# fixie-ai/ultravox

Measured on NVIDIA H100. Metric: audio-sec/s prefill (Llama-3.1-8B, 30s clip) at 1/2/4/8 H100; TTFT p50, higher is better.
Workload: dtype bf16

## Files before the change

### include/uvx.h

```cpp
#ifndef UVX_H_
#define UVX_H_

#include <stddef.h>
#include <stdint.h>

#ifdef __cplusplus
extern "C" {
#endif

#define UVX_ABI_VERSION 1

#define UVX_OK 0
#define UVX_ERR_ARG (-1)
#define UVX_ERR_CUDA (-2)
#define UVX_ERR_WS (-3)

typedef void* uvx_stream_t;

int uvx_abi_version(void);
const char* uvx_last_error(void);
int64_t uvx_launch_count(void);

size_t uvx_logmel_workspace(int64_t B, int64_t L, int n_mels);
int uvx_logmel(const float* wave, int64_t B, int64_t L, int n_mels, float* out_f32, void* out_tm,
               void* workspace, size_t workspace_bytes, uvx_stream_t stream);

int uvx_debug_mel_filters(int n_mels, float* host_dense);

int uvx_mel_to_timemajor(const float* mel, int64_t N, int n_mels, int64_t T, void* out_tm, uvx_stream_t stream);

enum { UVX_ACT_NONE = 0, UVX_ACT_GELU = 1, UVX_ACT_SWIGLU = 2 };
enum { UVX_DT_BF16 = 0, UVX_DT_F32 = 1 };
enum { UVX_TILE_PLAIN = 0, UVX_TILE_ROPE_PAIRS = 1, UVX_TILE_GATE_UP_8 = 8, UVX_TILE_GATE_UP_16 = 16 };

typedef struct uvx_gemm_args {
  const void* A;
  int64_t a_batch, a_rows, K;
  int64_t a_row_stride, a_batch_stride;
  const void* W;
  int64_t N, w_row_stride;
  void* C;
  int64_t c_row_stride, c_batch_rows, c_row_offset;
  const int32_t* c_row_map;
  const void* bias;
  const void* R;
  int64_t r_row_stride, r_batch_stride;
  float alpha;
  int32_t act;
  int32_t out_dtype;
  void* workspace;
  int64_t workspace_bytes;
  const void* norm_w;
  void* norm_out;
  float norm_eps;
  int32_t w_tiled;
  int32_t rope_cols;
  const float* rope_cos;
  const float* rope_sin;
  const int32_t* rope_positions;
  int64_t rope_rows_per_seq, rope_pos_offset;
  int32_t flags;
  int32_t w_perm;
} uvx_gemm_args;

int uvx_gemm_bf16(const uvx_gemm_args* args, uvx_stream_t stream);
int uvx_debug_gemm_override(int cfg, int splits);
int uvx_debug_gemm_stages(int n);
int uvx_debug_gemm_ws(int enable, int mode, int grid);
int uvx_debug_gemm_tma_store(int on);
int uvx_debug_gemm_times(void* dev_buf);
int uvx_debug_gemm_pf(int pf);
int uvx_debug_gemm_ws_times(void* dev_buf);
int uvx_tile_weight(const void* W, int64_t N, int64_t K, int64_t w_row_stride, int32_t R, int32_t interleave, void* out,
                    uvx_stream_t stream);
int uvx_debug_gemm_cluster(int cm, int cn);
int uvx_debug_gemm_mode(int mode);

int uvx_layernorm(const void* x, const void* w, const void* b, void* y, int64_t rows, int64_t cols,
                  int64_t x_row_stride, float eps, uvx_stream_t stream);
int uvx_rmsnorm(const void* x, const void* w, void* y, int64_t rows, int64_t cols, int64_t x_row_stride,
                int64_t group_rows, int64_t group_stride, int64_t valid_elems, float eps, uvx_stream_t stream);

typedef struct uvx_attn_args {
  const void *q, *k, *v;
  void* o;
  int64_t B, Hq, Hkv, Sq, Skv, D;
  int64_t q_rs, q_bs, k_rs, k_bs, v_rs, v_bs, o_rs, o_bs;
  const int32_t* kv_len;
  int32_t causal;
  int32_t block;
  float scale;
  float* lse;
// ... 144 lines not shown
```

### ultravox_b200/_lib.py

```python
from __future__ import annotations

import ctypes as C
import os
import pathlib

_HERE = pathlib.Path(__file__).resolve().parent
LIB_PATH = _HERE / "libuvx.so"

c_i64, c_i32, c_f32, c_vp, c_sz = C.c_int64, C.c_int32, C.c_float, C.c_void_p, C.c_size_t


class GemmArgs(C.Structure):
    _fields_ = [("A", c_vp), ("a_batch", c_i64), ("a_rows", c_i64), ("K", c_i64), ("a_row_stride", c_i64),
                ("a_batch_stride", c_i64), ("W", c_vp), ("N", c_i64), ("w_row_stride", c_i64), ("C", c_vp),
                ("c_row_stride", c_i64), ("c_batch_rows", c_i64), ("c_row_offset", c_i64), ("c_row_map", c_vp),
                ("bias", c_vp), ("R", c_vp), ("r_row_stride", c_i64), ("r_batch_stride", c_i64), ("alpha", c_f32),
                ("act", c_i32), ("out_dtype", c_i32), ("workspace", c_vp), ("workspace_bytes", c_i64),
                ("norm_w", c_vp), ("norm_out", c_vp), ("norm_eps", c_f32), ("w_tiled", c_i32), ("rope_cols", c_i32),
                ("rope_cos", c_vp), ("rope_sin", c_vp), ("rope_positions", c_vp), ("rope_rows_per_seq", c_i64),
                ("rope_pos_offset", c_i64), ("flags", c_i32), ("w_perm", c_i32)]


class AttnArgs(C.Structure):
    _fields_ = [("q", c_vp), ("k", c_vp), ("v", c_vp), ("o", c_vp), ("B", c_i64), ("Hq", c_i64), ("Hkv", c_i64),
# ... 7 lines not shown


class TensorList(C.Structure):
    _fields_ = [("count", c_i64), ("numel", c_i64 * TL_MAX), ("g", c_vp * TL_MAX), ("acc", c_vp * TL_MAX), ("p", c_vp * TL_MAX),
                ("m", c_vp * TL_MAX), ("v", c_vp * TL_MAX)]


SIGNATURES = {
    "uvx_abi_version": (C.c_int, []),
    "uvx_last_error": (C.c_char_p, []),
    "uvx_launch_count": (c_i64, []),
    "uvx_logmel_workspace": (c_sz, [c_i64, c_i64, C.c_int]),
    "uvx_logmel": (C.c_int, [c_vp, c_i64, c_i64, C.c_int, c_vp, c_vp, c_vp, c_sz, c_vp]),
    "uvx_debug_mel_filters": (C.c_int, [C.c_int, c_vp]),
    "uvx_mel_to_timemajor": (C.c_int, [c_vp, c_i64, C.c_int, c_i64, c_vp, c_vp]),
    "uvx_gemm_bf16": (C.c_int, [C.POINTER(GemmArgs), c_vp]),
    "uvx_debug_gemm_override": (C.c_int, [C.c_int, C.c_int]),
    "uvx_debug_gemm_cluster": (C.c_int, [C.c_int, C.c_int]),
    "uvx_debug_gemm_mode": (C.c_int, [C.c_int]),
    "uvx_debug_gemm_pf": (C.c_int, [C.c_int]),
    "uvx_debug_gemm_stages": (C.c_int, [C.c_int]),
    "uvx_debug_gemm_times": (C.c_int, [c_vp]),
    "uvx_debug_gemm_tma_store": (C.c_int, [C.c_int]),
    "uvx_debug_gemm_ws": (C.c_int, [C.c_int, C.c_int, C.c_int]),
    "uvx_debug_gemm_ws_times": (C.c_int, [C.c_void_p]),
    "uvx_tile_weight": (C.c_int, [c_vp, c_i64, c_i64, c_i64, c_i32, c_i32, c_vp, c_vp]),
    "uvx_layernorm": (C.c_int, [c_vp, c_vp, c_vp, c_vp, c_i64, c_i64, c_i64, c_f32, c_vp]),
    "uvx_rmsnorm": (C.c_int, [c_vp, c_vp, c_vp, c_i64, c_i64, c_i64, c_i64, c_i64, c_i64, c_f32, c_vp]),
    "uvx_attention": (C.c_int, [C.POINTER(AttnArgs), c_vp]),
    "uvx_debug_attn_tc": (C.c_int, [C.c_int]),
    "uvx_attention_enc_tc": (C.c_int, [c_vp, c_i64, c_i64, c_i64, c_i64, c_i64, c_i64, c_i64, c_vp, c_i64, c_vp, c_i32, c_f32, c_vp]),
    "uvx_attention_indexed": (C.c_int, [C.POINTER(AttnArgs), c_i64, c_vp, c_vp, c_vp]),
    "uvx_attention_paged": (C.c_int, [C.POINTER(AttnArgs), c_vp, c_i64, c_vp]),
    "uvx_attention_indexed_paged": (C.c_int, [C.POINTER(AttnArgs), c_i64, c_vp, c_i64, c_vp, c_vp, c_vp]),
    "uvx_kv_page_map": (C.c_int, [c_vp, c_i64, c_vp, c_vp, c_vp, c_i64, c_i64, c_vp, c_vp, c_vp]),
    "uvx_kv_pages_copy": (C.c_int, [c_vp, c_vp, c_i64, c_vp, c_vp, c_i64, c_i64, c_i64, c_vp, c_i64, c_i64, c_i32, c_vp]),
    "uvx_rope": (C.c_int, [c_vp, c_i64, c_i64, C.c_int, C.c_int, C.c_int, c_vp, c_vp, c_vp, c_i64, c_i64, c_vp]),
    "uvx_swiglu": (C.c_int, [c_vp, c_vp, c_i64, c_i64, c_i64, C.c_int, c_vp]),
    "uvx_splice_plan": (C.c_int, [c_vp, c_vp, c_vp, c_i64, c_i64, c_i64, c_i64, c_vp, c_vp]),
    "uvx_embed_splice": (C.c_int, [c_vp, c_vp, c_i64, c_vp, c_vp, c_i64, c_i64, c_vp, c_vp]),
    "uvx_lm_head": (C.c_int, [c_vp, c_i64, c_i64, c_vp, c_i64, c_i64, c_vp, c_vp]),
    "uvx_gemv_bf16": (C.c_int, [c_vp, c_i64, c_i64, c_vp, c_i64, c_i64, c_i64, c_vp, c_i64, c_vp, c_i64, C.c_int, c_vp]),
    "uvx_kv_append": (C.c_int, [c_vp, c_i64, c_i64, c_i64, c_i64, c_vp, c_vp, c_i64, c_vp, c_i64, c_vp]),
    "uvx_gemv_fused_bf16": (C.c_int, [c_vp, c_i64, c_i64, c_vp, c_i64, c_i64, c_i64, c_vp, c_i64, c_vp, c_i64, C.c_int, c_vp, C.c_float,
                                      C.c_int, c_vp]),
    "uvx_rope_kv_append": (C.c_int, [c_vp, c_i64, c_i64, C.c_int, C.c_int, C.c_int, c_vp, c_vp, c_vp, c_vp, c_vp, c_i64, c_vp, c_vp]),
# ... 74 lines not shown
```

### ultravox_b200/csrc/gemm_tc.cu

```cuda
#include <stdlib.h>

#include "uvx_common.cuh"
#include "tc_ptx.cuh"

namespace uvx {

struct GemmParams {
  int64_t a_rows, a_batch, K, N;
  void* C;
  int64_t c_row_stride, c_batch_rows, c_row_offset;
  const int32_t* c_row_map;
  const bf16* bias;
  const bf16* R;
  int64_t r_row_stride, r_batch_stride;
  float alpha;
  int act, out_f32;
  int m_tiles;
  int n_tiles, num_tiles;
  int splits, kb_per_split;
  float* ws_partial;
  const bf16* norm_w;
  bf16* norm_out;
  float norm_eps;
  int w_tiled;
  int w_perm;
  int swiglu;
  const float* rope_cos;
  const float* rope_sin;
  const int32_t* rope_pos;
  int64_t rope_rows_per_seq, rope_pos_offset;
  int rope_cols;
  int stages;
  int cm, cn;
  int staged_bytes;
  int r_bcast;
};

static constexpr int kSmemTotal = 227 * 1024;
static constexpr int kMaxStages = 8;
static constexpr int kGemmThreads = 384;
static constexpr int kPanelBytes = 128 * 128;

template <int MT, int BN>
struct WgLayout {
  static constexpr int kABytes = MT * 128 * kBK * 2;
  static constexpr int kWBytes = BN * kBK * 2;
  static constexpr int kStageBytes = kABytes + kWBytes;
  static constexpr int kRingMax = kSmemTotal - 1024 - 256;
  static constexpr int kStages = kRingMax / kStageBytes > kMaxStages ? kMaxStages : kRingMax / kStageBytes;
  static constexpr int kAcc = BN / 2;
  static_assert(kStages >= 2, "ring too shallow");
  static_assert(MT * kAcc <= 128, "accumulators must fit the register file");
};

__device__ __forceinline__ int tile_col(int tc, int perm) {
  if (!perm) return tc;
  const int q = tc >> 5, j = tc & 31;
  return j < 16 ? 16 * q + j : 64 + 16 * q + (j - 16);
}

__device__ __forceinline__ int64_t out_row(const GemmParams& p, int b, int64_t m) {
  return p.c_row_map ? (int64_t)p.c_row_map[(int64_t)b * p.a_rows + m] : (int64_t)b * p.c_batch_rows + m + p.c_row_offset;
}

template <int BN, int I>
__device__ __forceinline__ void swiglu_row(const GemmParams& p, const float* a, int h, int cq, bf16* crow, int64_t n_out0) {
#pragma unroll
  for (int j = 0; j < BN / 8; ++j) {
    if ((8 * j) % (2 * I) >= I) continue;
    const int64_t f = n_out0 + (8 * j / (2 * I)) * I + (8 * j) % (2 * I) + cq;
    if (f >= p.N / 2) continue;
// ... 8 lines not shown
    *reinterpret_cast<__nv_bfloat162*>(crow + f) = __floats2bfloat162_rn(o[0], o[1]);
  }
}

__device__ __forceinline__ void rope_store(const GemmParams& p, float x1a, float x1b, float x2a, float x2b, int64_t pos, int d, bf16* crow) {
  const float2 cs = *reinterpret_cast<const float2*>(p.rope_cos + pos * 64 + d);
  const float2 sn = *reinterpret_cast<const float2*>(p.rope_sin + pos * 64 + d);
  float o1a, o2a, o1b, o2b;
  rope_pair(__bfloat162float(__float2bfloat16_rn(x1a * p.alpha)), __bfloat162float(__float2bfloat16_rn(x2a * p.alpha)), cs.x, sn.x, o1a, o2a);
  rope_pair(__bfloat162float(__float2bfloat16_rn(x1b * p.alpha)), __bfloat162float(__float2bfloat16_rn(x2b * p.alpha)), cs.y, sn.y, o1b, o2b);
  *reinterpret_cast<__nv_bfloat162*>(crow + d) = __floats2bfloat162_rn(o1a, o1b);
  *reinterpret_cast<__nv_bfloat162*>(crow + d + 64) = __floats2bfloat162_rn(o2a, o2b);
}

template <int MT, int BN, bool STAGED>
__global__ void __launch_bounds__(kGemmThreads, 1)
gemm_wg_kernel(const __grid_constant__ CUtensorMap tmA, const __grid_constant__ CUtensorMap tmW, const __grid_constant__ CUtensorMap tmC,
               const __grid_constant__ CUtensorMap tmR, const GemmParams p) {
  using L = WgLayout<MT, BN>;
  static_assert(!STAGED || (MT == 1 && BN <= 128), "the staged epilogue is built for 128 x 64 and 128 x 128 tiles");
  pdl_trigger();
  extern __shared__ uint8_t smem_raw[];
  uint8_t* smem = (uint8_t*)(((uintptr_t)smem_raw + 1023) & ~(uintptr_t)1023);
  uint8_t* stage_c = smem + p.stages * L::kStageBytes;
  uint64_t* full_bar = (uint64_t*)(stage_c + p.staged_bytes);
  uint64_t* empty_bar = full_bar + kMaxStages;
  uint64_t* res_full = empty_bar + kMaxStages;
  uint64_t* stage_free = res_full + 1;

  const int wg = threadIdx.x >> 7, tid = threadIdx.x & 127;
  const int tiles_m_total = p.m_tiles * (int)p.a_batch;
  const int num_kb = (int)((p.K + kBK - 1) / kBK);
  const int stages = p.stages;
  const int cm = STAGED ? 1 : p.cm, cn = STAGED ? 1 : p.cn;
  const int csize = cm * cn;
  const int rank = csize > 1 ? (int)cluster_ctarank() : 0;
  const int rm = rank / cn, rn = rank % cn;
  const int cluster_tiles_m = tiles_m_total / cm;
  const int num_units = p.num_tiles / csize * p.splits;
  const int first_unit = blockIdx.x / csize, unit_step = gridDim.x / csize;

  if (threadIdx.x == 0) {
    for (int s = 0; s < stages; ++s) {
      mbar_init(&full_bar[s], 1);
      mbar_init(&empty_bar[s], 8 * csize);
    }
    if (STAGED) {
      mbar_init(res_full, 1);
      mbar_init(stage_free, 1);
    }
    asm volatile("fence.mbarrier_init.release.cluster;" ::: "memory");
    asm volatile("fence.proxy.async.shared::cta;" ::: "memory");
  }
  if (csize > 1) cluster_sync();
  else __syncthreads();
  pdl_wait();

  if (wg == 0) {
    asm volatile("setmaxnreg.dec.sync.aligned.u32 40;");
    if (tid == 0) {
      asm volatile("prefetch.tensormap [%0];" ::"l"(&tmA) : "memory");
      asm volatile("prefetch.tensormap [%0];" ::"l"(&tmW) : "memory");
      const int a_slice = MT * 128 / cn, w_slice = BN / cm;
      const uint16_t row_mask = (uint16_t)(((1u << cn) - 1u) << (rm * cn));
      uint16_t col_mask = 0;
      for (int j = 0; j < cm; ++j) col_mask |= (uint16_t)(1u << (j * cn + rn));
      int s = 0;
      uint32_t ph = 0;
      for (int unit = first_unit, tile_i = 0; unit < num_units; unit += unit_step, ++tile_i) {
        const int ctile = unit / p.splits, split = unit % p.splits;
        const int tm_idx = (ctile % cluster_tiles_m) * cm + rm;
        const int tn_idx = (ctile / cluster_tiles_m) * cn + rn;
        const int b = tm_idx / p.m_tiles;
        const int m0 = (tm_idx % p.m_tiles) * (MT * 128);
        const int kb_begin = split * p.kb_per_split;
        const int kb_end = min(num_kb, kb_begin + p.kb_per_split);
        const int wt_base = tn_idx * num_kb * BN;
        const int r_kb = max(kb_begin, kb_end - stages);
        for (int kb = kb_begin; kb < kb_end; ++kb) {
          mbar_wait(&empty_bar[s], ph ^ 1u);
          uint8_t* sa = smem + s * L::kStageBytes;
          mbar_expect_tx(&full_bar[s], (uint32_t)L::kStageBytes);
          uint8_t* da = sa + rn * a_slice * (kBK * 2);
          if (cn > 1) tma_load_3d_mc(da, &tmA, kb * kBK, m0 + rn * a_slice, b, &full_bar[s], row_mask);
          else tma_load_3d(da, &tmA, kb * kBK, m0, b, &full_bar[s]);
          uint8_t* dw = sa + L::kABytes + rm * w_slice * (kBK * 2);
          const int w0 = p.w_tiled ? 0 : kb * kBK;
          const int w1 = (p.w_tiled ? wt_base + kb * BN : tn_idx * BN) + rm * w_slice;
          if (cm > 1) tma_load_2d_mc(dw, &tmW, w0, w1, &full_bar[s], col_mask);
          else tma_load_2d(dw, &tmW, w0, w1, &full_bar[s]);
          if (++s == stages) { s = 0; ph ^= 1u; }
          if (STAGED && p.R && kb == r_kb) {
            mbar_wait(stage_free, (uint32_t)(tile_i & 1) ^ 1u);
            const int n0 = tn_idx * BN, panels = (int)min((int64_t)BN, p.N - n0) / 64;
            mbar_expect_tx(res_full, (uint32_t)(panels * kPanelBytes));
            for (int q = 0; q < panels; ++q) tma_load_3d(stage_c + q * kPanelBytes, &tmR, n0 + 64 * q, m0, p.r_bcast ? 0 : b, res_full);
          }
        }
      }
    }
    if (csize > 1) cluster_sync();
    return;
  }

  asm volatile("setmaxnreg.inc.sync.aligned.u32 232;");
  const int c = wg - 1;
  const int warp = tid >> 5, lane = tid & 31;
  auto release = [&](int slot) {
    __syncwarp();
    if (csize == 1) {
      if (lane == 0) mbar_arrive(&empty_bar[slot]);
    } else if (lane < csize) {
      mbar_arrive_cluster(&empty_bar[slot], (uint32_t)lane);
    }
  };
  auto store_thread = [&]() { return STAGED && threadIdx.x == 128; };
  int s = 0;
  uint32_t ph = 0;
  for (int unit = first_unit; unit < num_units; unit += unit_step) {
    const int ctile = unit / p.splits, split = unit % p.splits;
    const int tm_idx = (ctile % cluster_tiles_m) * cm + rm;
    const int tn_idx = (ctile / cluster_tiles_m) * cn + rn;
    const int b = tm_idx / p.m_tiles;
    const int m0 = (tm_idx % p.m_tiles) * (MT * 128);
    const int n0 = tn_idx * BN;
    const int kb_begin = split * p.kb_per_split;
    const int kb_end = min(num_kb, kb_begin + p.kb_per_split);

    float acc[MT][L::kAcc];
    int prev = -1;
    for (int kb = kb_begin; kb < kb_end; ++kb) {
      mbar_wait(&full_bar[s], ph);
      const uint32_t sa = smem_u32(smem + s * L::kStageBytes);
      const uint64_t dw = make_wgmma_desc(sa + L::kABytes);
      wgmma_fence();
#pragma unroll
      for (int mt = 0; mt < MT; ++mt) {
        const uint64_t da = make_wgmma_desc(sa + (mt * 128 + c * 64) * (kBK * 2));
#pragma unroll
        for (int k = 0; k < kBK / 16; ++k)
          Wgmma<BN>::mma(acc[mt], da + (uint64_t)(2 * k), dw + (uint64_t)(2 * k), (kb > kb_begin || k > 0) ? 1u : 0u);
      }
      wgmma_commit();
      if (store_thread() && kb == kb_begin && unit != first_unit) {
        bulk_wait_read0();
        mbar_arrive(stage_free);
      }
      wgmma_wait<1>();
      if (prev >= 0) release(prev);
      prev = s;
      if (++s == stages) { s = 0; ph ^= 1u; }
    }
    wgmma_wait<0>();
    release(prev);

    const int rq = warp * 16 + (lane >> 2);
    const int cq = 2 * (lane & 3);
    if constexpr (STAGED) {
      {
        const uint32_t tile_par = (uint32_t)((unit - first_unit) / unit_step) & 1u;
        if (p.R) mbar_wait(res_full, tile_par);
        else mbar_wait(stage_free, tile_par ^ 1u);
        __nv_bfloat162 bias_v[BN / 8];
#pragma unroll
        for (int j = 0; j < BN / 8; ++j) {
          const int64_t n = n0 + 8 * j + cq;
          if (p.bias && n < p.N) bias_v[j] = *reinterpret_cast<const __nv_bfloat162*>(p.bias + n);
        }
        const uint32_t st0 = smem_u32(stage_c);
#pragma unroll
        for (int h = 0; h < 2; ++h) {
          const int r = c * 64 + rq + 8 * h;
          const uint32_t row = st0 + (uint32_t)r * 128u, sw = (uint32_t)(r & 7);
#pragma unroll
          for (int j = 0; j < BN / 8; ++j) {
            float v0 = acc[0][4 * j + 2 * h] * p.alpha, v1 = acc[0][4 * j + 2 * h + 1] * p.alpha;
            if (p.bias) {
// ... 455 lines not shown
                   CU_TENSOR_MAP_INTERLEAVE_NONE, CU_TENSOR_MAP_SWIZZLE_128B, promo, CU_TENSOR_MAP_FLOAT_OOB_FILL_NONE);
  if (r != CUDA_SUCCESS) {
    set_error("cuTensorMapEncodeTiled failed with CUresult %d (rank %d dims %llu %llu stride %llu)", (int)r, rank,
              (unsigned long long)dims[0], (unsigned long long)dims[1], (unsigned long long)strides_bytes[0]);
    return UVX_ERR_CUDA;
  }
  return UVX_OK;
}

static int num_sms() {
  static int n = 0;
  if (!n) {
    int dev = 0;
    cudaGetDevice(&dev);
    cudaDeviceGetAttribute(&n, cudaDevAttrMultiProcessorCount, dev);
    if (n <= 0) n = 132;
  }
  return n;
}

static int g_gemm_stage_cap = 0;
static int g_grid_cap = 0;
static int g_tma_store = -1;

static int finish_gemm(const uvx_gemm_args* a, const GemmParams& p, cudaStream_t stream) {
  const bool want_norm = a->norm_w && a->norm_out;
  if (p.splits == 1) {
    if (!want_norm) return UVX_OK;
    return uvx_rmsnorm(a->C, a->norm_w, a->norm_out, a->a_batch * a->a_rows, a->N, a->c_row_stride, 0, 0, 0, a->norm_eps, stream);
  }
  if (want_norm && !p.out_f32 && a->N <= 8192 && !a->c_row_map && a->act == UVX_ACT_NONE) {
    launch_k(splitk_reduce_rmsnorm_kernel, dim3((unsigned)(a->a_batch * a->a_rows)), dim3(256), 0, stream, p);
    return check_launch("splitk_reduce_rmsnorm_kernel");
  }
  const int64_t total = a->a_batch * a->a_rows * (a->N / 8);
  int64_t blocks = (total + 255) / 256;
  if (blocks > (int64_t)num_sms() * 8) blocks = (int64_t)num_sms() * 8;
  launch_k(splitk_reduce_kernel, dim3((unsigned)blocks), dim3(256), 0, stream, p);
  int rc = check_launch("splitk_reduce_kernel");
  if (rc || !want_norm) return rc;
  return uvx_rmsnorm(a->C, a->norm_w, a->norm_out, a->a_batch * a->a_rows, a->N, a->c_row_stride, 0, 0, 0, a->norm_eps, stream);
}

static void legal_cluster(int mt, int bn, int tiles_m_total, int n_tiles, int* cm, int* cn) {
  if (*cm < 1 || *cm > 4 || tiles_m_total % *cm != 0 || bn % (8 * *cm) != 0) *cm = 1;
  if (*cn < 1 || *cn > 4 || n_tiles % *cn != 0 || (mt * 128) % (8 * *cn) != 0) *cn = 1;
  if (*cm * *cn > 8) *cm = *cn = 1;
}

template <int MT, int BN, bool STAGED>
static cudaError_t set_smem_attr() {
  if constexpr (STAGED && !(MT == 1 && BN <= 128)) return cudaErrorInvalidValue;
  else return cudaFuncSetAttribute(gemm_wg_kernel<MT, BN, STAGED>, cudaFuncAttributeMaxDynamicSharedMemorySize, kSmemTotal);
}

template <int MT, int BN>
static int launch_gemm(const uvx_gemm_args* a, int splits, int cm, int cn, cudaStream_t stream) {
  using L = WgLayout<MT, BN>;
  const int m_tiles = (int)((a->a_rows + MT * 128 - 1) / (MT * 128));
  const int n_tiles = (int)((a->N + BN - 1) / BN);
  legal_cluster(MT, BN, m_tiles * (int)a->a_batch, n_tiles, &cm, &cn);
  CUtensorMap tmA, tmW;
  {
    uint64_t dims[3] = {(uint64_t)a->K, (uint64_t)a->a_rows, (uint64_t)a->a_batch};
    uint64_t st[2] = {(uint64_t)a->a_row_stride * 2, (uint64_t)(a->a_batch > 1 ? a->a_batch_stride : a->a_row_stride) * 2};
    uint32_t box[3] = {kBK, (uint32_t)(MT * 128 / cn), 1};
    int rc = encode_map(&tmA, a->A, 3, dims, st, box, CU_TENSOR_MAP_L2_PROMOTION_L2_128B);
    if (rc) return rc;
  }
  const bool tiled = a->w_tiled != 0;
  if (tiled) {
    UVX_REQUIRE(a->w_tiled == BN && a->K % kBK == 0, "uvx_gemm_bf16: tiled weights need BN == tile rows and K %% 64 == 0");
    const uint64_t n_tiles_w = (uint64_t)((a->N + BN - 1) / BN);
    uint64_t dims[2] = {(uint64_t)kBK, n_tiles_w * (uint64_t)(a->K / kBK) * (uint64_t)BN};
    uint64_t st[1] = {(uint64_t)kBK * 2};
    uint32_t box[2] = {kBK, (uint32_t)(BN / cm)};
    int rc = encode_map(&tmW, a->W, 2, dims, st, box, CU_TENSOR_MAP_L2_PROMOTION_L2_256B);
    if (rc) return rc;
  } else {
    uint64_t dims[2] = {(uint64_t)a->K, (uint64_t)a->N};
    uint64_t st[1] = {(uint64_t)a->w_row_stride * 2};
    uint32_t box[2] = {kBK, (uint32_t)(BN / cm)};
    int rc = encode_map(&tmW, a->W, 2, dims, st, box, CU_TENSOR_MAP_L2_PROMOTION_L2_256B);
    if (rc) return rc;
  }
  GemmParams p;
  memset(&p, 0, sizeof(p));
  p.w_tiled = tiled ? 1 : 0;
  p.w_perm = a->w_perm == 1 ? 1 : 0;
// ... 9 lines not shown
  p.a_batch = a->a_batch;
  p.K = a->K;
  p.N = a->N;
  p.C = a->C;
  p.c_row_stride = a->c_row_stride;
  p.c_batch_rows = a->c_batch_rows;
  p.c_row_offset = a->c_row_offset;
  p.c_row_map = a->c_row_map;
  p.bias = (const bf16*)a->bias;
  p.R = (const bf16*)a->R;
  p.r_row_stride = a->r_row_stride;
  p.r_batch_stride = a->r_batch_stride;
  p.alpha = a->alpha;
  p.act = a->act;
  p.out_f32 = a->out_dtype == UVX_DT_F32;
  p.norm_w = (const bf16*)a->norm_w;
  p.norm_out = (bf16*)a->norm_out;
  p.norm_eps = a->norm_eps;
  p.m_tiles = m_tiles;
  p.n_tiles = n_tiles;
  p.num_tiles = p.m_tiles * (int)a->a_batch * p.n_tiles;
  p.cm = cm;
  p.cn = cn;
  const int num_kb = (int)((a->K + kBK - 1) / kBK);
  if (a->N % BN != 0) splits = 1;
  const size_t per_split = (size_t)a->a_batch * (size_t)a->a_rows * (size_t)a->N * 4;
  while (splits > 1 && (!a->workspace || per_split * (size_t)splits > (size_t)a->workspace_bytes)) --splits;
  if (splits > num_kb) splits = num_kb;
  if (splits < 1) splits = 1;
  p.kb_per_split = (num_kb + splits - 1) / splits;
  p.splits = (num_kb + p.kb_per_split - 1) / p.kb_per_split;
  p.ws_partial = (float*)a->workspace;
  CUtensorMap tmC, tmR;
  memset(&tmC, 0, sizeof(tmC));
  memset(&tmR, 0, sizeof(tmR));
  const bool staged = MT == 1 && BN <= 128 && g_tma_store != 0 && (a->a_rows > 256 || a->a_batch > 1) && p.splits == 1 &&
                      cm * cn == 1 && !a->c_row_map && !p.swiglu && !p.rope_cos && !p.w_perm && !(a->norm_w && a->norm_out) &&
                      (!a->R || (!p.out_f32 && a->r_row_stride > 0 && (uintptr_t)a->R % 16 == 0));
  if (staged) {
    const uint64_t es = p.out_f32 ? 4 : 2;
    const uint64_t row_bytes = (uint64_t)a->c_row_stride * es;
    uint64_t dims[3] = {(uint64_t)a->N, (uint64_t)a->a_rows, (uint64_t)a->a_batch};
    uint64_t st[2] = {row_bytes, a->a_batch > 1 ? (uint64_t)a->c_batch_rows * row_bytes : row_bytes};
    uint32_t box[3] = {(uint32_t)(128 / es), 128, 1};
    int rc = encode_map(&tmC, (const char*)a->C + a->c_row_offset * (int64_t)row_bytes, 3, dims, st, box,
                        CU_TENSOR_MAP_L2_PROMOTION_NONE, p.out_f32 ? CU_TENSOR_MAP_DATA_TYPE_FLOAT32 : CU_TENSOR_MAP_DATA_TYPE_BFLOAT16);
    if (rc) return rc;
    if (a->R) {
      p.r_bcast = a->a_batch == 1 || a->r_batch_stride == 0;
      uint64_t rdims[3] = {(uint64_t)a->N, (uint64_t)a->a_rows, p.r_bcast ? 1 : (uint64_t)a->a_batch};
      uint64_t rst[2] = {(uint64_t)a->r_row_stride * 2, (uint64_t)(p.r_bcast ? a->r_row_stride : a->r_batch_stride) * 2};
      uint32_t rbox[3] = {64, 128, 1};
      rc = encode_map(&tmR, a->R, 3, rdims, rst, rbox, CU_TENSOR_MAP_L2_PROMOTION_L2_128B);
      if (rc) return rc;
    }
    p.staged_bytes = BN / 64 * (p.out_f32 ? 2 : 1) * kPanelBytes;
  }
  p.stages = (L::kRingMax - p.staged_bytes) / L::kStageBytes;
  if (p.stages > L::kStages) p.stages = L::kStages;
  if (g_gemm_stage_cap >= 2 && p.stages > g_gemm_stage_cap) p.stages = g_gemm_stage_cap;
  const int smem = p.stages * L::kStageBytes + p.staged_bytes + 1024 + 2 * kMaxStages * 8 + 16;
  static bool attr_set[2] = {false, false};
  if (!attr_set[staged]) {
    cudaError_t e = staged ? set_smem_attr<MT, BN, true>() : set_smem_attr<MT, BN, false>();
    if (e != cudaSuccess) {
      set_error("cudaFuncSetAttribute(gemm_wg_kernel<%d,%d,%d>, smem %d): %s", MT, BN, (int)staged, kSmemTotal, cudaGetErrorString(e));
      return UVX_ERR_CUDA;
    }
    attr_set[staged] = true;
  }
  const int csize = cm * cn;
  const int units = p.num_tiles / csize * p.splits;
  int max_units = num_sms();
  if (csize > 1) {
    static int max_clusters[9] = {0};
    if (!max_clusters[csize]) {
      cudaLaunchConfig_t cfg = {};
      cfg.gridDim = dim3((unsigned)csize);
      cfg.blockDim = dim3(kGemmThreads);
      cfg.dynamicSmemBytes = (size_t)smem;
      cudaLaunchAttribute attr;
      attr.id = cudaLaunchAttributeClusterDimension;
      attr.val.clusterDim.x = (unsigned)csize;
      attr.val.clusterDim.y = 1;
// ... 159 lines not shown
extern "C" int uvx_debug_gemm_stages(int n) {
  uvx::g_gemm_stage_cap = n;
  return UVX_OK;
}

extern "C" int uvx_debug_gemm_ws(int enable, int mode, int grid) {
  (void)mode;
  uvx::g_ws_enable = enable;
  uvx::g_grid_cap = grid > 0 ? grid : 0;
  return UVX_OK;
}

static int forced_cm = 0, forced_cn = 0;
static int g_cluster_enable = -1;

extern "C" int uvx_debug_gemm_cluster(int cm, int cn) {
  forced_cm = cm;
  forced_cn = cn;
  return UVX_OK;
}

extern "C" int uvx_debug_gemm_tma_store(int on) {
  uvx::g_tma_store = on;
  return UVX_OK;
}

extern "C" int uvx_debug_gemm_mode(int mode) { (void)mode; return UVX_OK; }
extern "C" int uvx_debug_gemm_times(void* dev_buf) { (void)dev_buf; return UVX_OK; }
extern "C" int uvx_debug_gemm_pf(int pf) { (void)pf; return UVX_OK; }
extern "C" int uvx_debug_gemm_ws_times(void* dev_buf) { (void)dev_buf; return UVX_OK; }

static void read_forced() {
  if (forced < 0) {
    const char* e = getenv("UVX_GEMM_CFG");
    forced = e ? atoi(e) : 0;
    const char* s = getenv("UVX_GEMM_SPLITS");
    forced_splits = s ? atoi(s) : 0;
  }
}

static void pick_cfg(int64_t rows, int64_t batch, int64_t N, int64_t K, int sms, int* mt_out, int* bn_out, int* splits) {
  const int num_kb = (int)((K + 63) / 64);
  int mt, bn;
  if (rows <= 256 && batch == 1) {
    mt = rows > 128 ? 2 : 1;
    bn = N % 128 == 0 ? 128 : 64;
// ... 107 lines not shown
```

### ultravox_b200/model.py

```python
from __future__ import annotations

import dataclasses
import os
from typing import Optional

import torch
import torch.nn as nn
from transformers.modeling_outputs import CausalLMOutputWithPast

from . import ops
from .config import LossConfig, LossFunction, UltravoxConfig

FUSE_NORM = os.environ.get("UVX_FUSE_NORM", "1") != "0"
USE_TILED = os.environ.get("UVX_TILED", "1") != "0"
FUSE_ROPE = os.environ.get("UVX_FUSE_ROPE", "1") != "0"
QKV_MODE = os.environ.get("UVX_QKV_MODE", "fused")
TILED_SET = os.environ.get("UVX_TILED_SET", "gate_up")
USE_WS = os.environ.get("UVX_GEMM_WS", "0") == "1"
FUSE_SWIGLU = os.environ.get("UVX_FUSE_SWIGLU", "1") != "0"
BF16 = torch.bfloat16


class _P(nn.Module):

# ... 378 lines not shown
    @torch.no_grad()
    def _tiled_weights(self):
        if getattr(self, "_tiled", None) is None:
            self._tiled = False
            layers = self.language_model.model.layers
            if USE_TILED and len(layers) > 0 and layers[0].self_attn.qkv_w.is_cuda:
                tc = self.config.text_config
                hs, ffn = tc.hidden_size, tc.intermediate_size
                per_layer = 2 * (layers[0].self_attn.qkv_w.numel() + hs * layers[0].self_attn.o_proj.weight.shape[1] + 3 * hs * ffn)
                free, _ = torch.cuda.mem_get_info(self.device)
                if hs % 64 == 0 and ffn % 64 == 0 and ffn % 8 == 0 and free > 1.15 * per_layer * len(layers) + (8 << 30):
                    out = []
                    for layer in layers:
                        sa, mlp = layer.self_attn, layer.mlp
                        attn_t = USE_WS or TILED_SET == "all"
                        down_t = USE_WS or TILED_SET in ("all", "mlp")
                        gu_rows = 128
                        lm_hd = self.language_model.head_dim
                        out.append(dict(qkv=ops.TiledWeight(sa.qkv_w, 128, rope_pairs=USE_WS and lm_hd == 128) if attn_t else None,
                                        o=ops.TiledWeight(sa.o_proj.weight, 128) if attn_t else None,
                                        gate_up=ops.TiledWeight(mlp.gate_up_w, gu_rows, swiglu=True) if FUSE_SWIGLU
                                        else ops.TiledWeight(mlp.gate_up_w, gu_rows),
                                        down=ops.TiledWeight(mlp.down_proj.weight, 128) if down_t else None))
                    self._tiled = out
        return self._tiled or None

    def _rope_tables(self, need: int):
        have = 0 if self._rope is None else self._rope[0].shape[0]
        if have < need:
            cap = int(getattr(self.config.text_config, "max_position_embeddings", 0) or 0)
            n = max(need, 4096, 2 * have)
            if cap >= need:
                n = min(n, cap)
            self._rope = ops.rope_tables(self._inv_freq, n, self.device)
        return self._rope

    def encode_audio(self, x_tm: torch.Tensor, audio_lens: Optional[torch.Tensor],
                     kv_len: Optional[torch.Tensor] = None) -> torch.Tensor:
        at = self.audio_tower
        N, Tp, _ = x_tm.shape
        T = Tp - 2
        if T > at.max_context_length:
            raise ValueError(f"Whisper expects the mel input features to be of length {at.max_context_length} or less, "
                             f"but found {T}. Make sure to pad the input mel features to {at.max_context_length}.")
        d, H = at.d, at.heads
        T2 = (T + 1) // 2
# ... 91 lines not shown
        dev = inputs_embeds.device
        past = cache.length if cache is not None else 0
        cos, sin = self._rope_tables(past + S)
        h = inputs_embeds.view(B * S, Dm)
        x = torch.empty_like(h)
        qkv = torch.empty(B * S, (nq + 2 * nkv) * hd, dtype=BF16, device=dev)
        att = torch.empty(B * S, nq * hd, dtype=BF16, device=dev)
        ffn = tc.intermediate_size
        tiled = self._tiled_weights()
        if USE_WS and B * S > 256:
            tiled = None
        fuse_act = tiled is not None and tiled[0]["gate_up"].swiglu
        gu = None if fuse_act else torch.empty(B * S, 2 * ffn, dtype=BF16, device=dev)
        act = torch.empty(B * S, ffn, dtype=BF16, device=dev)
        rs = qkv.stride(0)
        layers = lm.model.layers
        rope = (cos, sin, positions, S, past, (nq + nkv) * hd) if (FUSE_ROPE and QKV_MODE == "fused" and hd == 128) else None
        qkv_flags = 1 if QKV_MODE == "r1" else 0
        ops.rmsnorm(h, layers[0].input_layernorm.weight, eps, out=x)
        for li, layer in enumerate(layers):
            sa, mlp = layer.self_attn, layer.mlp
            tw = tiled[li] if tiled is not None else None
            if tw is not None and tw["qkv"] is not None:
                ops.linear_tiled(x, tw["qkv"], out=qkv, rope=rope)
            else:
                ops.linear(x, sa.qkv_w, out=qkv, rope=rope, flags=qkv_flags)
            if rope is None:
                ops.rope_(qkv, nq, nkv, hd, cos, sin, rows_per_seq=S, pos_offset=past, positions=positions)
            if cache is None:
                ops.attention_fused_qkv(qkv, B, S, nq, nkv, hd, hd ** -0.5, True, kv_len, 0, out=att, kv_start=kv_start)
            else:
                kc, vc = cache.k[li], cache.v[li]
                ops.kv_write(qkv, kc, vc, B, S, past, nq, nkv, hd)
                smax = kc.shape[1]
                ops.attention(qkv.data_ptr(), kc.data_ptr(), vc.data_ptr(), att, B, nq, nkv, S, past + S, hd,
                              (rs, S * rs, nkv * hd, smax * nkv * hd, nkv * hd, smax * nkv * hd, nq * hd, S * nq * hd),
                              hd ** -0.5, True, kv_len, 0, kv_start)
            n1 = (layer.post_attention_layernorm.weight, eps, x) if FUSE_NORM else None
            if tw is not None and tw["o"] is not None:
                ops.linear_tiled(att, tw["o"], residual=h, out=h, norm=n1)
            else:
                ops.linear(att, sa.o_proj.weight, residual=h, out=h, norm=n1)
            if not FUSE_NORM:
                ops.rmsnorm(h, layer.post_attention_layernorm.weight, eps, out=x)
            if fuse_act:
                ops.linear_tiled(x, tw["gate_up"], out=act, act=ops.ACT_SWIGLU)
            else:
                if tw is not None:
                    ops.linear_tiled(x, tw["gate_up"], out=gu)
                else:
                    ops.linear(x, mlp.gate_up_w, out=gu)
                ops.swiglu(gu, gate_first=True, out=act)
            nxt = layers[li + 1].input_layernorm.weight if li + 1 < len(layers) else lm.model.norm.weight
            n2 = (nxt, eps, x) if FUSE_NORM else None
            if tw is not None and tw["down"] is not None:
                ops.linear_tiled(act, tw["down"], residual=h, out=h, norm=n2)
            else:
                ops.linear(act, mlp.down_proj.weight, residual=h, out=h, norm=n2)
            if not FUSE_NORM:
                ops.rmsnorm(h, nxt, eps, out=x)
        if cache is not None:
            cache.length = past + S
        return x.view(B, S, Dm)

    def load_state_dict(self, state_dict, strict: bool = True, _track: bool = True, **kwargs):
        import re
        from . import lora
        if lora.has_lora_keys(state_dict):
            scaling = {"audio_tower": lora.lora_scaling(getattr(self.config, "audio_model_lora_config", None)),
                       "language_model": lora.lora_scaling(getattr(self.config, "text_model_lora_config", None))}
            state_dict = lora.merge_lora_state_dict(state_dict, scaling)
        if self.language_model.tied and "language_model.lm_head.weight" not in state_dict \
                and "language_model.model.embed_tokens.weight" in state_dict:
            state_dict = dict(state_dict)
            state_dict["language_model.lm_head.weight"] = state_dict["language_model.model.embed_tokens.weight"]
        if _track:
            self.keep_params.update(state_dict.keys())
        res = super().load_state_dict(state_dict, strict=False, **kwargs)
        ignorable = [re.compile(p.replace(".", r"\.").replace("*", ".*")) for p in self._keys_to_ignore_on_load_missing]
# ... 338 lines not shown
```

### ultravox_b200/ops.py

```python
from __future__ import annotations

import ctypes as C
import math
from typing import Optional

import torch

from . import _lib
from ._lib import AttnArgs, GemmArgs, check, lib

ACT_NONE, ACT_GELU = 0, 1
BF16 = torch.bfloat16


def _stream() -> int:
    return torch.cuda.current_stream().cuda_stream


def _cuda(t: torch.Tensor, dtype=None, name="tensor") -> torch.Tensor:
    if not t.is_cuda:
        raise _lib.UvxError(f"{name} must be a CUDA tensor (ultravox_b200 has no CPU path)")
    if dtype is not None and t.dtype != dtype:
        raise TypeError(f"{name} must be {dtype}, got {t.dtype}")
    return t
# ... 80 lines not shown
        a.rope_rows_per_seq, a.rope_pos_offset, a.rope_cols = int(rows_per_seq), int(pos_offset), int(rope_cols)
    check(lib().uvx_gemm_bf16(C.byref(a), _stream()), "uvx_gemm_bf16")


class TiledWeight:

    def __init__(self, w: torch.Tensor, R: int, swiglu: bool = False, rope_pairs: bool = False):
        _cuda(w, BF16, "w")
        self.N, self.K, self.R, self.swiglu = int(w.shape[0]), int(w.shape[1]), int(R), bool(swiglu)
        self.rope_pairs = bool(rope_pairs)
        if rope_pairs and (swiglu or R != 128 or self.N % 128 != 0):
            raise ValueError("rope_pairs: a 128-row image of whole 128-wide heads")
        n_tiles = -(-self.N // R)
        self.image = torch.empty(n_tiles * (self.K // 64) * R * 64, dtype=BF16, device=w.device)
        inter = ((16 if R == 128 else 8) if swiglu else (1 if rope_pairs else 0))
        check(lib().uvx_tile_weight(w.data_ptr(), self.N, self.K, w.stride(0), R, inter, self.image.data_ptr(), _stream()), "uvx_tile_weight")

    @property
    def n_out(self) -> int:
        return self.N // 2 if self.swiglu else self.N


ACT_SWIGLU = 2


def linear_tiled(x: torch.Tensor, wt: TiledWeight, out: Optional[torch.Tensor] = None, residual: Optional[torch.Tensor] = None,
                 act: int = ACT_NONE, norm: Optional[tuple] = None, rope: Optional[tuple] = None) -> torch.Tensor:
    _cuda(x, BF16, "x")
    K = x.shape[-1]
    x2 = x.reshape(-1, K)
    if x2.stride(-1) != 1:
        x2 = x2.contiguous()
    M = x2.shape[0]
    n_out = wt.n_out if act == ACT_SWIGLU else wt.N
    if (act == ACT_SWIGLU) != wt.swiglu:
        raise ValueError("ACT_SWIGLU needs (and only works with) the gate|up-interleaved weight image")
    if out is None:
        out = torch.empty(*x.shape[:-1], n_out, dtype=BF16, device=x.device)
    o2 = out.view(-1, n_out)
    a = GemmArgs()
    a.A, a.a_batch, a.a_rows, a.K = x2.data_ptr(), 1, M, K
    a.a_row_stride, a.a_batch_stride = x2.stride(0), 0
    a.W, a.N, a.w_row_stride = wt.image.data_ptr(), wt.N, K
    a.C, a.c_row_stride, a.c_batch_rows, a.c_row_offset = o2.data_ptr(), o2.stride(0), M, 0
    if residual is not None:
        r2 = residual.reshape(-1, n_out)
        a.R, a.r_row_stride = r2.data_ptr(), r2.stride(0)
    a.alpha, a.act, a.out_dtype = 1.0, act, 0
    ws = gemm_workspace(out.device)
    a.workspace, a.workspace_bytes = ws.data_ptr(), ws.numel()
    if norm is not None:
        a.norm_w, a.norm_eps, a.norm_out = norm[0].data_ptr(), float(norm[1]), norm[2].data_ptr()
    a.w_tiled = wt.R
    a.w_perm = 1 if wt.rope_pairs else 0
    if rope is not None:
        cos, sin, positions, rows_per_seq, pos_offset, rope_cols = rope
        a.rope_cos, a.rope_sin, a.rope_positions = cos.data_ptr(), sin.data_ptr(), _p(positions)
        a.rope_rows_per_seq, a.rope_pos_offset, a.rope_cols = int(rows_per_seq), int(pos_offset), int(rope_cols)
    check(lib().uvx_gemm_bf16(C.byref(a), _stream()), "uvx_gemm_bf16(tiled)")
    return out


def linear(x: torch.Tensor, w: torch.Tensor, bias: Optional[torch.Tensor] = None, act: int = ACT_NONE,
           residual: Optional[torch.Tensor] = None, out: Optional[torch.Tensor] = None,
           out_dtype=BF16, row_map: Optional[torch.Tensor] = None, alpha: float = 1.0,
           norm: Optional[tuple] = None, rope: Optional[tuple] = None, flags: int = 0) -> torch.Tensor:
    _cuda(x, BF16, "x"), _cuda(w, BF16, "w")
    K = x.shape[-1]
    x2 = x.reshape(-1, K)
    if x2.stride(-1) != 1:
        x2 = x2.contiguous()
    M, N = x2.shape[0], w.shape[0]
    if out is None:
        out = torch.empty(*x.shape[:-1], N, dtype=out_dtype, device=x.device)
    o2 = out.view(-1, out.shape[-1]) if row_map is None else out
    r2 = None
    if residual is not None:
# ... 720 lines not shown
```

Before: 1824.

## Split GEMM smem ring into separate A and W rings with early weight prefetch

For small-M GEMMs (single M tile, BN≤128, non-staged), shared memory is split into a small A ring sized to the actual row count and a deeper W ring. Separate producer lanes and mbarriers drive each ring. For weights flagged static, the W producer issues its first loads before the PDL grid-dependency wait, so weight streaming overlaps the previous kernel's tail. A host sync is also added after weight tiling so the early loads cannot read an incomplete image. This deepens the weight prefetch pipeline for memory-bound skinny GEMMs, at the cost of more barrier state and extra complexity in the producer and consumer loops.

```diff
diff --git a/include/uvx.h b/include/uvx.h
--- a/include/uvx.h
+++ b/include/uvx.h
@@ -32,6 +32,7 @@
 enum { UVX_ACT_NONE = 0, UVX_ACT_GELU = 1, UVX_ACT_SWIGLU = 2 };
 enum { UVX_DT_BF16 = 0, UVX_DT_F32 = 1 };
 enum { UVX_TILE_PLAIN = 0, UVX_TILE_ROPE_PAIRS = 1, UVX_TILE_GATE_UP_8 = 8, UVX_TILE_GATE_UP_16 = 16 };
+enum { UVX_GEMM_W_STATIC = 4 };
 
 typedef struct uvx_gemm_args {
   const void* A;
@@ -68,6 +69,7 @@
 int uvx_debug_gemm_stages(int n);
 int uvx_debug_gemm_ws(int enable, int mode, int grid);
 int uvx_debug_gemm_tma_store(int on);
+int uvx_debug_gemm_split_ring(int a_stages);
 int uvx_debug_gemm_times(void* dev_buf);
 int uvx_debug_gemm_pf(int pf);
 int uvx_debug_gemm_ws_times(void* dev_buf);
diff --git a/ultravox_b200/_lib.py b/ultravox_b200/_lib.py
--- a/ultravox_b200/_lib.py
+++ b/ultravox_b200/_lib.py
@@ -53,6 +53,7 @@
     "uvx_debug_gemm_stages": (C.c_int, [C.c_int]),
     "uvx_debug_gemm_times": (C.c_int, [c_vp]),
     "uvx_debug_gemm_tma_store": (C.c_int, [C.c_int]),
+    "uvx_debug_gemm_split_ring": (C.c_int, [C.c_int]),
     "uvx_debug_gemm_ws": (C.c_int, [C.c_int, C.c_int, C.c_int]),
     "uvx_debug_gemm_ws_times": (C.c_int, [C.c_void_p]),
     "uvx_tile_weight": (C.c_int, [c_vp, c_i64, c_i64, c_i64, c_i32, c_i32, c_vp, c_vp]),
diff --git a/ultravox_b200/csrc/gemm_tc.cu b/ultravox_b200/csrc/gemm_tc.cu
--- a/ultravox_b200/csrc/gemm_tc.cu
+++ b/ultravox_b200/csrc/gemm_tc.cu
@@ -31,6 +31,9 @@
   int64_t rope_rows_per_seq, rope_pos_offset;
   int rope_cols;
   int stages;
+  int a_stages;
+  int a_box_rows;
+  int w_early;
   int cm, cn;
   int staged_bytes;
   int r_bcast;
@@ -38,6 +41,10 @@
 
 static constexpr int kSmemTotal = 227 * 1024;
 static constexpr int kMaxStages = 8;
+static constexpr int kMaxWStages = 16;
+static constexpr int kMaxAStages = 8;
+static constexpr int kBarBytes = 512;
+static_assert((2 * kMaxWStages + 2 + 2 * kMaxAStages) * 8 <= kBarBytes, "barrier region");
 static constexpr int kGemmThreads = 384;
 static constexpr int kPanelBytes = 128 * 128;
 
@@ -46,7 +53,7 @@
   static constexpr int kABytes = MT * 128 * kBK * 2;
   static constexpr int kWBytes = BN * kBK * 2;
   static constexpr int kStageBytes = kABytes + kWBytes;
-  static constexpr int kRingMax = kSmemTotal - 1024 - 256;
+  static constexpr int kRingMax = kSmemTotal - 1024 - kBarBytes;
   static constexpr int kStages = kRingMax / kStageBytes > kMaxStages ? kMaxStages : kRingMax / kStageBytes;
   static constexpr int kAcc = BN / 2;
   static_assert(kStages >= 2, "ring too shallow");
@@ -101,16 +108,23 @@
   pdl_trigger();
   extern __shared__ uint8_t smem_raw[];
   uint8_t* smem = (uint8_t*)(((uintptr_t)smem_raw + 1023) & ~(uintptr_t)1023);
-  uint8_t* stage_c = smem + p.stages * L::kStageBytes;
+  constexpr bool kSplitRing = !STAGED && BN <= 128;
+  const bool split_ring = kSplitRing && p.a_stages > 0;
+  const int stages = p.stages, a_stages = split_ring ? p.a_stages : stages;
+  const int a_box_bytes = p.a_box_rows * (kBK * 2);
+  const int a_stride = split_ring ? a_box_bytes : L::kStageBytes, w_stride = split_ring ? L::kWBytes : L::kStageBytes;
+  uint8_t* const w_ring = split_ring ? smem + a_stages * a_box_bytes : smem + L::kABytes;
+  uint8_t* stage_c = smem + (split_ring ? a_stages * a_box_bytes + stages * L::kWBytes : stages * L::kStageBytes);
   uint64_t* full_bar = (uint64_t*)(stage_c + p.staged_bytes);
-  uint64_t* empty_bar = full_bar + kMaxStages;
-  uint64_t* res_full = empty_bar + kMaxStages;
+  uint64_t* empty_bar = full_bar + kMaxWStages;
+  uint64_t* res_full = empty_bar + kMaxWStages;
   uint64_t* stage_free = res_full + 1;
+  uint64_t* const a_full = split_ring ? stage_free + 1 : full_bar;
+  uint64_t* const a_empty = split_ring ? a_full + kMaxAStages : empty_bar;
 
   const int wg = threadIdx.x >> 7, tid = threadIdx.x & 127;
   const int tiles_m_total = p.m_tiles * (int)p.a_batch;
   const int num_kb = (int)((p.K + kBK - 1) / kBK);
-  const int stages = p.stages;
   const int cm = STAGED ? 1 : p.cm, cn = STAGED ? 1 : p.cn;
   const int csize = cm * cn;
   const int rank = csize > 1 ? (int)cluster_ctarank() : 0;
@@ -124,6 +138,12 @@
       mbar_init(&full_bar[s], 1);
       mbar_init(&empty_bar[s], 8 * csize);
     }
+    if (split_ring) {
+      for (int s = 0; s < a_stages; ++s) {
+        mbar_init(&a_full[s], 1);
+        mbar_init(&a_empty[s], 8 * csize);
+      }
+    }
     if (STAGED) {
       mbar_init(res_full, 1);
       mbar_init(stage_free, 1);
@@ -133,19 +153,22 @@
   }
   if (csize > 1) cluster_sync();
   else __syncthreads();
-  pdl_wait();
+  const bool w_lane = wg == 0 && tid == 0, a_lane = split_ring && wg == 0 && tid == 32;
+  const bool w_early = split_ring && p.w_early && w_lane;
+  if (!w_early) pdl_wait();
 
   if (wg == 0) {
     asm volatile("setmaxnreg.dec.sync.aligned.u32 40;");
-    if (tid == 0) {
-      asm volatile("prefetch.tensormap [%0];" ::"l"(&tmA) : "memory");
-      asm volatile("prefetch.tensormap [%0];" ::"l"(&tmW) : "memory");
-      const int a_slice = MT * 128 / cn, w_slice = BN / cm;
+    if (w_lane || a_lane) {
+      const bool do_w = w_lane, do_a = split_ring ? a_lane : w_lane;
+      if (do_a) asm volatile("prefetch.tensormap [%0];" ::"l"(&tmA) : "memory");
+      if (do_w) asm volatile("prefetch.tensormap [%0];" ::"l"(&tmW) : "memory");
+      const int a_slice = p.a_box_rows / cn, w_slice = BN / cm;
       const uint16_t row_mask = (uint16_t)(((1u << cn) - 1u) << (rm * cn));
       uint16_t col_mask = 0;
       for (int j = 0; j < cm; ++j) col_mask |= (uint16_t)(1u << (j * cn + rn));
-      int s = 0;
-      uint32_t ph = 0;
+      int s = 0, sa = 0, issued = 0;
+      uint32_t ph = 0, pha = 0;
       for (int unit = first_unit, tile_i = 0; unit < num_units; unit += unit_step, ++tile_i) {
         const int ctile = unit / p.splits, split = unit % p.splits;
         const int tm_idx = (ctile % cluster_tiles_m) * cm + rm;
@@ -157,18 +180,29 @@
         const int wt_base = tn_idx * num_kb * BN;
         const int r_kb = max(kb_begin, kb_end - stages);
         for (int kb = kb_begin; kb < kb_end; ++kb) {
-          mbar_wait(&empty_bar[s], ph ^ 1u);
-          uint8_t* sa = smem + s * L::kStageBytes;
-          mbar_expect_tx(&full_bar[s], (uint32_t)L::kStageBytes);
-          uint8_t* da = sa + rn * a_slice * (kBK * 2);
-          if (cn > 1) tma_load_3d_mc(da, &tmA, kb * kBK, m0 + rn * a_slice, b, &full_bar[s], row_mask);
-          else tma_load_3d(da, &tmA, kb * kBK, m0, b, &full_bar[s]);
-          uint8_t* dw = sa + L::kABytes + rm * w_slice * (kBK * 2);
-          const int w0 = p.w_tiled ? 0 : kb * kBK;
-          const int w1 = (p.w_tiled ? wt_base + kb * BN : tn_idx * BN) + rm * w_slice;
-          if (cm > 1) tma_load_2d_mc(dw, &tmW, w0, w1, &full_bar[s], col_mask);
-          else tma_load_2d(dw, &tmW, w0, w1, &full_bar[s]);
+          if (do_w) {
+            if (w_early && issued++ == stages) pdl_wait();
+            mbar_wait(&empty_bar[s], ph ^ 1u);
+            mbar_expect_tx(&full_bar[s], (uint32_t)(split_ring ? L::kWBytes : L::kStageBytes));
+          }
+          if (do_a) {
+            if (split_ring) {
+              mbar_wait(&a_empty[sa], pha ^ 1u);
+              mbar_expect_tx(&a_full[sa], (uint32_t)a_box_bytes);
+            }
+            uint8_t* da = smem + sa * a_stride + rn * a_slice * (kBK * 2);
+            if (cn > 1) tma_load_3d_mc(da, &tmA, kb * kBK, m0 + rn * a_slice, b, &a_full[sa], row_mask);
+            else tma_load_3d(da, &tmA, kb * kBK, m0, b, &a_full[sa]);
+          }
+          if (do_w) {
+            uint8_t* dw = w_ring + s * w_stride + rm * w_slice * (kBK * 2);
+            const int w0 = p.w_tiled ? 0 : kb * kBK;
+            const int w1 = (p.w_tiled ? wt_base + kb * BN : tn_idx * BN) + rm * w_slice;
+            if (cm > 1) tma_load_2d_mc(dw, &tmW, w0, w1, &full_bar[s], col_mask);
+            else tma_load_2d(dw, &tmW, w0, w1, &full_bar[s]);
+          }
           if (++s == stages) { s = 0; ph ^= 1u; }
+          if (++sa == a_stages) { sa = 0; pha ^= 1u; }
           if (STAGED && p.R && kb == r_kb) {
             mbar_wait(stage_free, (uint32_t)(tile_i & 1) ^ 1u);
             const int n0 = tn_idx * BN, panels = (int)min((int64_t)BN, p.N - n0) / 64;
@@ -185,17 +219,17 @@
   asm volatile("setmaxnreg.inc.sync.aligned.u32 232;");
   const int c = wg - 1;
   const int warp = tid >> 5, lane = tid & 31;
-  auto release = [&](int slot) {
+  auto release = [&](uint64_t* bar) {
     __syncwarp();
     if (csize == 1) {
-      if (lane == 0) mbar_arrive(&empty_bar[slot]);
+      if (lane == 0) mbar_arrive(bar);
     } else if (lane < csize) {
-      mbar_arrive_cluster(&empty_bar[slot], (uint32_t)lane);
+      mbar_arrive_cluster(bar, (uint32_t)lane);
     }
   };
   auto store_thread = [&]() { return STAGED && threadIdx.x == 128; };
-  int s = 0;
-  uint32_t ph = 0;
+  int s = 0, sa = 0;
+  uint32_t ph = 0, pha = 0;
   for (int unit = first_unit; unit < num_units; unit += unit_step) {
     const int ctile = unit / p.splits, split = unit % p.splits;
     const int tm_idx = (ctile % cluster_tiles_m) * cm + rm;
@@ -207,15 +241,16 @@
     const int kb_end = min(num_kb, kb_begin + p.kb_per_split);
 
     float acc[MT][L::kAcc];
-    int prev = -1;
+    int prev = -1, prev_a = -1;
     for (int kb = kb_begin; kb < kb_end; ++kb) {
       mbar_wait(&full_bar[s], ph);
-      const uint32_t sa = smem_u32(smem + s * L::kStageBytes);
-      const uint64_t dw = make_wgmma_desc(sa + L::kABytes);
+      if (split_ring) mbar_wait(&a_full[sa], pha);
+      const uint32_t a_addr = smem_u32(smem + sa * a_stride);
+      const uint64_t dw = make_wgmma_desc(smem_u32(w_ring + s * w_stride));
       wgmma_fence();
 #pragma unroll
       for (int mt = 0; mt < MT; ++mt) {
-        const uint64_t da = make_wgmma_desc(sa + (mt * 128 + c * 64) * (kBK * 2));
+        const uint64_t da = make_wgmma_desc(a_addr + (mt * 128 + c * 64) * (kBK * 2));
 #pragma unroll
         for (int k = 0; k < kBK / 16; ++k)
           Wgmma<BN>::mma(acc[mt], da + (uint64_t)(2 * k), dw + (uint64_t)(2 * k), (kb > kb_begin || k > 0) ? 1u : 0u);
@@ -226,12 +261,18 @@
         mbar_arrive(stage_free);
       }
       wgmma_wait<1>();
-      if (prev >= 0) release(prev);
+      if (prev >= 0) {
+        release(&empty_bar[prev]);
+        if (split_ring) release(&a_empty[prev_a]);
+      }
       prev = s;
+      prev_a = sa;
       if (++s == stages) { s = 0; ph ^= 1u; }
+      if (++sa == a_stages) { sa = 0; pha ^= 1u; }
     }
     wgmma_wait<0>();
-    release(prev);
+    release(&empty_bar[prev]);
+    if (split_ring) release(&a_empty[prev_a]);
 
     const int rq = warp * 16 + (lane >> 2);
     const int cq = 2 * (lane & 3);
@@ -733,6 +774,7 @@
 static int g_gemm_stage_cap = 0;
 static int g_grid_cap = 0;
 static int g_tma_store = -1;
+static int g_split_ring = -1;
 
 static int finish_gemm(const uvx_gemm_args* a, const GemmParams& p, cudaStream_t stream) {
   const bool want_norm = a->norm_w && a->norm_out;
@@ -771,11 +813,19 @@
   const int m_tiles = (int)((a->a_rows + MT * 128 - 1) / (MT * 128));
   const int n_tiles = (int)((a->N + BN - 1) / BN);
   legal_cluster(MT, BN, m_tiles * (int)a->a_batch, n_tiles, &cm, &cn);
+  const int box_rows = (int)((a->a_rows + 7) / 8 * 8);
+  int split_a = g_split_ring > 0 ? (g_split_ring < kMaxAStages ? g_split_ring : kMaxAStages) : 5;
+  if (split_a < 2) split_a = 2;
+  int split_w = (L::kRingMax - split_a * box_rows * kBK * 2) / L::kWBytes;
+  if (split_w > kMaxWStages) split_w = kMaxWStages;
+  const bool split_ring = BN <= 128 && g_split_ring != 0 && a->a_batch == 1 && m_tiles == 1 && cn == 1 &&
+                          (g_split_ring > 0 || split_w > L::kStages);
+  const int a_box_rows = split_ring ? box_rows : MT * 128;
   CUtensorMap tmA, tmW;
   {
     uint64_t dims[3] = {(uint64_t)a->K, (uint64_t)a->a_rows, (uint64_t)a->a_batch};
     uint64_t st[2] = {(uint64_t)a->a_row_stride * 2, (uint64_t)(a->a_batch > 1 ? a->a_batch_stride : a->a_row_stride) * 2};
-    uint32_t box[3] = {kBK, (uint32_t)(MT * 128 / cn), 1};
+    uint32_t box[3] = {kBK, (uint32_t)(a_box_rows / cn), 1};
     int rc = encode_map(&tmA, a->A, 3, dims, st, box, CU_TENSOR_MAP_L2_PROMOTION_L2_128B);
     if (rc) return rc;
   }
@@ -831,6 +881,7 @@
   p.num_tiles = p.m_tiles * (int)a->a_batch * p.n_tiles;
   p.cm = cm;
   p.cn = cn;
+  p.a_box_rows = a_box_rows;
   const int num_kb = (int)((a->K + kBK - 1) / kBK);
   if (a->N % BN != 0) splits = 1;
   const size_t per_split = (size_t)a->a_batch * (size_t)a->a_rows * (size_t)a->N * 4;
@@ -865,10 +916,22 @@
     }
     p.staged_bytes = BN / 64 * (p.out_f32 ? 2 : 1) * kPanelBytes;
   }
-  p.stages = (L::kRingMax - p.staged_bytes) / L::kStageBytes;
-  if (p.stages > L::kStages) p.stages = L::kStages;
-  if (g_gemm_stage_cap >= 2 && p.stages > g_gemm_stage_cap) p.stages = g_gemm_stage_cap;
-  const int smem = p.stages * L::kStageBytes + p.staged_bytes + 1024 + 2 * kMaxStages * 8 + 16;
+  int ring_bytes;
+  if (split_ring) {
+    const int a_bytes = a_box_rows * kBK * 2;
+    p.a_stages = split_a;
+    p.stages = split_w;
+    if (g_gemm_stage_cap >= 2 && p.stages > g_gemm_stage_cap) p.stages = g_gemm_stage_cap;
+    UVX_REQUIRE(p.stages >= 2 && (MT * 128 - a_box_rows) * kBK * 2 <= p.stages * L::kWBytes, "uvx_gemm_bf16: split ring does not fit");
+    p.w_early = (a->flags & UVX_GEMM_W_STATIC) ? 1 : 0;
+    ring_bytes = p.a_stages * a_bytes + p.stages * L::kWBytes;
+  } else {
+    p.stages = (L::kRingMax - p.staged_bytes) / L::kStageBytes;
+    if (p.stages > L::kStages) p.stages = L::kStages;
+    if (g_gemm_stage_cap >= 2 && p.stages > g_gemm_stage_cap) p.stages = g_gemm_stage_cap;
+    ring_bytes = p.stages * L::kStageBytes;
+  }
+  const int smem = ring_bytes + p.staged_bytes + 1024 + kBarBytes;
   static bool attr_set[2] = {false, false};
   if (!attr_set[staged]) {
     cudaError_t e = staged ? set_smem_attr<MT, BN, true>() : set_smem_attr<MT, BN, false>();
@@ -1074,6 +1137,11 @@
 
 extern "C" int uvx_debug_gemm_tma_store(int on) {
   uvx::g_tma_store = on;
+  return UVX_OK;
+}
+
+extern "C" int uvx_debug_gemm_split_ring(int a_stages) {
+  uvx::g_split_ring = a_stages;
   return UVX_OK;
 }
 
diff --git a/ultravox_b200/model.py b/ultravox_b200/model.py
--- a/ultravox_b200/model.py
+++ b/ultravox_b200/model.py
@@ -424,6 +424,8 @@
                                         gate_up=ops.TiledWeight(mlp.gate_up_w, gu_rows, swiglu=True) if FUSE_SWIGLU
                                         else ops.TiledWeight(mlp.gate_up_w, gu_rows),
                                         down=ops.TiledWeight(mlp.down_proj.weight, 128) if down_t else None))
+                    if not torch.cuda.is_current_stream_capturing():
+                        torch.cuda.current_stream(self.device).synchronize()
                     self._tiled = out
         return self._tiled or None
 
@@ -561,7 +563,7 @@
             sa, mlp = layer.self_attn, layer.mlp
             tw = tiled[li] if tiled is not None else None
             if tw is not None and tw["qkv"] is not None:
-                ops.linear_tiled(x, tw["qkv"], out=qkv, rope=rope)
+                ops.linear_tiled(x, tw["qkv"], out=qkv, rope=rope, flags=ops.GEMM_W_STATIC)
             else:
                 ops.linear(x, sa.qkv_w, out=qkv, rope=rope, flags=qkv_flags)
             if rope is None:
@@ -577,23 +579,23 @@
                               hd ** -0.5, True, kv_len, 0, kv_start)
             n1 = (layer.post_attention_layernorm.weight, eps, x) if FUSE_NORM else None
             if tw is not None and tw["o"] is not None:
-                ops.linear_tiled(att, tw["o"], residual=h, out=h, norm=n1)
+                ops.linear_tiled(att, tw["o"], residual=h, out=h, norm=n1, flags=ops.GEMM_W_STATIC)
             else:
                 ops.linear(att, sa.o_proj.weight, residual=h, out=h, norm=n1)
             if not FUSE_NORM:
                 ops.rmsnorm(h, layer.post_attention_layernorm.weight, eps, out=x)
             if fuse_act:
-                ops.linear_tiled(x, tw["gate_up"], out=act, act=ops.ACT_SWIGLU)
+                ops.linear_tiled(x, tw["gate_up"], out=act, act=ops.ACT_SWIGLU, flags=ops.GEMM_W_STATIC)
             else:
                 if tw is not None:
-                    ops.linear_tiled(x, tw["gate_up"], out=gu)
+                    ops.linear_tiled(x, tw["gate_up"], out=gu, flags=ops.GEMM_W_STATIC)
                 else:
                     ops.linear(x, mlp.gate_up_w, out=gu)
                 ops.swiglu(gu, gate_first=True, out=act)
             nxt = layers[li + 1].input_layernorm.weight if li + 1 < len(layers) else lm.model.norm.weight
             n2 = (nxt, eps, x) if FUSE_NORM else None
             if tw is not None and tw["down"] is not None:
-                ops.linear_tiled(act, tw["down"], residual=h, out=h, norm=n2)
+                ops.linear_tiled(act, tw["down"], residual=h, out=h, norm=n2, flags=ops.GEMM_W_STATIC)
             else:
                 ops.linear(act, mlp.down_proj.weight, residual=h, out=h, norm=n2)
             if not FUSE_NORM:
diff --git a/ultravox_b200/ops.py b/ultravox_b200/ops.py
--- a/ultravox_b200/ops.py
+++ b/ultravox_b200/ops.py
@@ -126,10 +126,11 @@
 
 
 ACT_SWIGLU = 2
+GEMM_W_STATIC = 4
 
 
 def linear_tiled(x: torch.Tensor, wt: TiledWeight, out: Optional[torch.Tensor] = None, residual: Optional[torch.Tensor] = None,
-                 act: int = ACT_NONE, norm: Optional[tuple] = None, rope: Optional[tuple] = None) -> torch.Tensor:
+                 act: int = ACT_NONE, norm: Optional[tuple] = None, rope: Optional[tuple] = None, flags: int = 0) -> torch.Tensor:
     _cuda(x, BF16, "x")
     K = x.shape[-1]
     x2 = x.reshape(-1, K)
@@ -157,6 +158,7 @@
         a.norm_w, a.norm_eps, a.norm_out = norm[0].data_ptr(), float(norm[1]), norm[2].data_ptr()
     a.w_tiled = wt.R
     a.w_perm = 1 if wt.rope_pairs else 0
+    a.flags = flags
     if rope is not None:
         cos, sin, positions, rows_per_seq, pos_offset, rope_cols = rope
         a.rope_cos, a.rope_sin, a.rope_positions = cos.data_ptr(), sin.data_ptr(), _p(positions)
```

Measured after the change: 1882, median of 6. 1.03x the previous value.
